# harukaki/brl

Measured on AMD Instinct MI355X. Metric: env-steps/sec at num_envs=8192, 32-step rollout, 1/2/4/8 MI355X, higher is better.
Workload: dtype u8

## Files before the change

brl_amd/csrc/brl_mlp_gemm_x3.hip:

```cpp
#include <hip/hip_runtime.h>
#include <stdint.h>

#include "abi_common.hpp"
#include "mlp_gemm_x3.hpp"
#include "mlp_linear_x3p.hpp"

static int64_t x3_tiles(int64_t m, int64_t n) { return ((m + 127) / 128) * ((n + 127) / 128); }

static int64_t x3_workspace_bytes(int64_t m, int64_t n, int64_t k) {
  const int sk = mgs::pick_splitk(m, n, k);
  if (sk == 1) return 0;
  const int64_t tiles = x3_tiles(m, n);
  return ((tiles * 4 + 255) / 256) * 256 + tiles * sk * (int64_t)mgs::SLAB_FLOATS * 4;
}

extern "C" int brl_mlp_gemm_x3_workspace(int64_t m, int64_t n, int64_t k, int64_t *bytes) {
  NEED(bytes && m > 0 && n > 0 && k > 0, "bytes / m / n / k");
  *bytes = x3_workspace_bytes(m, n, k);
  return BRL_OK;
}

extern "C" int brl_mlp_gemm_x3(int device, int layout, int epilogue, const float *a, int64_t lda, const float *b, int64_t ldb, float *c,
                               int64_t ldc, int64_t m, int64_t n, int64_t k, int act, const float *bias, const float *gate, int64_t ldg,
                               float *colsum, void *workspace, int64_t workspace_bytes, void *stream) {
  NEED(a && b && c && m > 0 && n > 0 && k > 0, "a / b / c / m / n / k");
  NEED(layout >= BRL_GEMM_NT && layout <= BRL_GEMM_TN, "layout (BRL_GEMM_NT / _NN / _TN)");
  NEED(m < (1 << 24) && n < (1 << 24) && k < (1 << 24), "m / n / k below 2^24");
  NEED(n % 4 == 0 && ldc % 4 == 0 && lda % 4 == 0 && ldb % 4 == 0 && ldc >= n, "n and the leading dimensions multiples of 4 (16-byte pieces)");
  const bool akc = layout != BRL_GEMM_TN, bkc = layout == BRL_GEMM_NT;
  NEED(k % 32 == 0, "k a multiple of 32 (whole 32-deep chunks; other k: brl_mlp_gemm)");
  NEED(akc ? lda >= k : lda >= ((m + 3) & ~(int64_t)3), "lda (where m is contiguous in a: at least m rounded up to 4 — whole 16-byte pieces are read)");
  NEED(bkc ? ldb >= k : ldb >= n, "ldb");
  NEED((akc ? m * lda : k * lda) < (1ll << 29) && (bkc ? n * ldb : k * ldb) < (1ll << 29), "operands below 2 GB");
  NEED(act == 0 || act == 1, "act (0 ReLU, 1 tanh)");
  NEED((epilogue == BRL_GEMM_EPI_NONE) || (epilogue == BRL_GEMM_EPI_BIAS_ACT && layout == BRL_GEMM_NT && bias) ||
           (epilogue == BRL_GEMM_EPI_GATE_COLSUM && layout == BRL_GEMM_NN && gate && ldg >= n && ldg % 4 == 0),
       "epilogue (NONE; BIAS_ACT with NT + bias; GATE_COLSUM with NN + gate)");
  NEED((((uintptr_t)a | (uintptr_t)b | (uintptr_t)c | (uintptr_t)bias | (uintptr_t)gate | (uintptr_t)colsum) & 15) == 0, "16-byte alignment");
  HIP_TRY(hipSetDevice(device));
  mgs::Args X{};
  mg::Args &G = X.g;
  G.A = a; G.lda = lda; G.B = b; G.ldb = ldb; G.C = c; G.ldc = ldc;
  G.M = (int)m; G.N = (int)n; G.K = (int)k; G.act = act;
  G.bias = bias; G.gate = gate; G.ldg = ldg; G.colsum = colsum;
  const int64_t tiles = x3_tiles(m, n);
  int sk = mgs::pick_splitk(m, n, k);
  const int64_t tick = ((tiles * 4 + 255) / 256) * 256;
  if (sk > 1 && (workspace == nullptr || workspace_bytes < tick + tiles * sk * (int64_t)mgs::SLAB_FLOATS * 4)) sk = 1;
  NEED(sk == 1 || (((uintptr_t)workspace) & 255) == 0, "workspace: 256-byte alignment");
  NEED(sk == 1 || tiles * sk * (int64_t)mgs::SLAB_FLOATS * 4 < (1ll << 31), "partial tiles below 2 GB");
  X.splitk = sk;
  X.tickets = (unsigned *)workspace;
  X.slabs = sk > 1 ? (float *)((char *)workspace + tick) : nullptr;
  const unsigned blocks = (unsigned)(tiles * sk);
  hipStream_t s = (hipStream_t)stream;
#define X3_LAUNCH(AK, BK_, E) hipLaunchKernelGGL((mgs::k_gemm_x3s<AK, BK_, E>), dim3(blocks), dim3(mgs::THREADS), 0, s, X)
  if (layout == BRL_GEMM_NT) {
    if (epilogue == BRL_GEMM_EPI_BIAS_ACT) X3_LAUNCH(true, true, mg::EPI_BIAS_ACT);
    else X3_LAUNCH(true, true, mg::EPI_NONE);
  } else if (layout == BRL_GEMM_NN) {
    if (epilogue == BRL_GEMM_EPI_GATE_COLSUM) X3_LAUNCH(true, false, mg::EPI_GATE_COLSUM);
    else X3_LAUNCH(true, false, mg::EPI_NONE);
  } else {
    X3_LAUNCH(false, false, mg::EPI_NONE);
  }
#undef X3_LAUNCH
  HIP_TRY(hipGetLastError());
  return BRL_OK;
}

extern "C" int brl_mlp_gemm_x3_group(int device, int layout, int count, const float *const *a, const int64_t *lda, const float *const *b,
                                     const int64_t *ldb, float *const *c, const int64_t *ldc, const int64_t *m, const int64_t *n,
                                     const int64_t *k, void *stream) {
  NEED(count >= 1 && count <= mgs::GROUP_MAX && a && lda && b && ldb && c && ldc && m && n && k, "count (1..8) / NULL array");
  NEED(layout >= BRL_GEMM_NT && layout <= BRL_GEMM_TN, "layout (BRL_GEMM_NT / _NN / _TN)");
  const bool akc = layout != BRL_GEMM_TN, bkc = layout == BRL_GEMM_NT;
  mgs::GroupArgs GA{};
  GA.n = count;
  for (int i = 0; i < count; i++) {
    NEED(a[i] && b[i] && c[i] && m[i] > 0 && n[i] > 0 && k[i] > 0, "a / b / c / m / n / k");
    NEED(m[i] < (1 << 24) && n[i] < (1 << 24) && k[i] < (1 << 24), "m / n / k below 2^24");
    NEED(n[i] % 4 == 0 && ldc[i] % 4 == 0 && lda[i] % 4 == 0 && ldb[i] % 4 == 0 && ldc[i] >= n[i], "n and the leading dimensions multiples of 4");
    NEED(k[i] % 32 == 0, "k a multiple of 32 (whole 32-deep chunks; other k: brl_mlp_gemm_group)");
    NEED(akc ? lda[i] >= k[i] : lda[i] >= ((m[i] + 3) & ~(int64_t)3), "lda (where m is contiguous in a: at least m rounded up to 4)");
    NEED(bkc ? ldb[i] >= k[i] : ldb[i] >= n[i], "ldb");
    NEED((akc ? m[i] * lda[i] : k[i] * lda[i]) < (1ll << 29) && (bkc ? n[i] * ldb[i] : k[i] * ldb[i]) < (1ll << 29), "operands below 2 GB");
    NEED((((uintptr_t)a[i] | (uintptr_t)b[i] | (uintptr_t)c[i]) & 15) == 0, "16-byte alignment");
    mgs::Args &X = GA.x[i];
    mg::Args &G = X.g;
    G.A = a[i]; G.lda = lda[i]; G.B = b[i]; G.ldb = ldb[i]; G.C = c[i]; G.ldc = ldc[i];
    G.M = (int)m[i]; G.N = (int)n[i]; G.K = (int)k[i];
    X.splitk = 1;
    GA.first[i + 1] = GA.first[i] + (int)x3_tiles(m[i], n[i]);
  }
  HIP_TRY(hipSetDevice(device));
  hipStream_t s = (hipStream_t)stream;
  const unsigned blocks = (unsigned)GA.first[count];
  if (layout == BRL_GEMM_NT) hipLaunchKernelGGL((mgs::k_gemm_x3s_group<true, true>), dim3(blocks), dim3(mgs::THREADS), 0, s, GA);
  else if (layout == BRL_GEMM_NN) hipLaunchKernelGGL((mgs::k_gemm_x3s_group<true, false>), dim3(blocks), dim3(mgs::THREADS), 0, s, GA);
  else hipLaunchKernelGGL((mgs::k_gemm_x3s_group<false, false>), dim3(blocks), dim3(mgs::THREADS), 0, s, GA);
  HIP_TRY(hipGetLastError());
  return BRL_OK;
}

extern "C" int brl_split_planes(int device, const float *x, int64_t n, uint16_t *planes, int64_t plane_stride, void *stream) {
  NEED(x && planes && n > 0 && n % 4 == 0 && plane_stride >= n && plane_stride % 4 == 0, "x / planes / n (a multiple of 4) / plane_stride");
  NEED((((uintptr_t)x) & 15) == 0 && (((uintptr_t)planes) & 7) == 0, "alignment (x 16 bytes, planes 8)");
  HIP_TRY(hipSetDevice(device));
  hipLaunchKernelGGL(lx3::k_split_planes, dim3((unsigned)((n / 4 + 255) / 256)), dim3(256), 0, (hipStream_t)stream, x, planes, plane_stride, n / 4);
  HIP_TRY(hipGetLastError());
  return BRL_OK;
}

extern "C" int brl_linear_x3p(int device, const uint16_t *x_planes, int npx, int64_t ldx, int64_t sx, const uint16_t *w_planes, int64_t ldw,
                              int64_t sw, const float *bias, int relu, float *y, int64_t ldy, uint16_t *y_planes, int64_t ldyp, int64_t syp,
                              int64_t m, int64_t n, int64_t k, void *stream) {
  NEED(x_planes && w_planes && bias && (y || y_planes) && m > 0 && n > 0 && k > 0, "x_planes / w_planes / bias / an output / m / n / k");
  NEED(npx == 1 || npx == 3, "npx (3 planes, or 1: x exact in bf16)");
  NEED(n % 128 == 0 && k % 32 == 0, "n a multiple of 128, k a multiple of 32");
  NEED(m < (1 << 24) && n < (1 << 24) && k < (1 << 24), "m / n / k below 2^24");
  NEED(ldx >= k && ldx % 8 == 0 && ldw >= k && ldw % 8 == 0, "ldx / ldw (at least k, multiples of 8: 16-byte pieces)");
  NEED(m * ldx < (1ll << 31) && n * ldw < (1ll << 31), "planes below 4 GB each");
  NEED(!y || (ldy >= n && ldy % 4 == 0), "ldy");
  NEED(!y_planes || (ldyp >= n && ldyp % 8 == 0 && syp % 8 == 0), "ldyp / syp (multiples of 8)");
  NEED(sx % 8 == 0 && sw % 8 == 0, "plane strides multiples of 8");
  NEED((((uintptr_t)x_planes | (uintptr_t)w_planes | (uintptr_t)bias | (uintptr_t)y | (uintptr_t)y_planes) & 15) == 0, "16-byte alignment");
  HIP_TRY(hipSetDevice(device));
  lx3::Args G{};
  G.x = x_planes; G.ldx = ldx; G.sx = sx; G.w = w_planes; G.ldw = ldw; G.sw = sw; G.bias = bias;
  G.y = y; G.ldy = ldy; G.yp = y_planes; G.ldyp = ldyp; G.syp = syp;
  G.M = (int)m; G.N = (int)n; G.K = (int)k; G.relu = relu ? 1 : 0;
  hipStream_t s = (hipStream_t)stream;
  const unsigned blocks = (unsigned)(((m + 127) / 128) * (n / 128));
  if (npx == 3) hipLaunchKernelGGL(lx3::k_linear_x3p<3>, dim3(blocks), dim3(lx3::THREADS), 0, s, G);
  else hipLaunchKernelGGL(lx3::k_linear_x3p<1>, dim3(blocks), dim3(lx3::THREADS), 0, s, G);
  HIP_TRY(hipGetLastError());
  return BRL_OK;
}
```

brl_amd/csrc/mlp_linear_x3p.hpp:

```cpp
#pragma once

#include "mlp_gemm.hpp"

namespace lx3 {

using mg::f32x4;
typedef __bf16 bf16x8 __attribute__((ext_vector_type(8)));
typedef float f32x16 __attribute__((ext_vector_type(16)));
typedef unsigned u32x4 __attribute__((ext_vector_type(4)));
typedef unsigned u32x2 __attribute__((ext_vector_type(2)));

constexpr int BK = 32, STAGES = 3, THREADS = 512;
constexpr int PLANE = 128 * 64;
constexpr int STAGE_BYTES = 6 * PLANE;
constexpr int LDS_BYTES = STAGES * STAGE_BYTES;
constexpr int C_ROW_BYTES = 128 * 2 + 16;
static_assert(3 * 128 * C_ROW_BYTES <= LDS_BYTES, "the output planes reuse the stages");

struct Args {
  const uint16_t *x;
  int64_t ldx, sx;
  const uint16_t *w;
  int64_t ldw, sw;
  const float *bias;
  float *y;
  int64_t ldy;
  uint16_t *yp;
  int64_t ldyp, syp;
  int M, N, K;
  int relu;
#ifdef LX3_TIMING
  unsigned long long *dbg;
#endif
};
#ifdef LX3_TIMING
#define LX3_STAMP(k) do { if (threadIdx.x == 0 && G.dbg) { G.dbg[(size_t)blockIdx.x * 4 + 2 * (k)] = __builtin_amdgcn_s_memtime(); \
                                                          G.dbg[(size_t)blockIdx.x * 4 + 2 * (k) + 1] = __builtin_amdgcn_s_memrealtime(); } } while (0)
#else
#define LX3_STAMP(k) do { } while (0)
#endif

template <bool V>
struct BoolTag { static constexpr bool value = V; };

#ifndef LX3_STORE
#define LX3_STORE 0
#endif
#ifndef LX3_EXP
#define LX3_EXP 0
#endif

__device__ __forceinline__ void glds16(const void *g, void *lds_wave_base) {
  __builtin_amdgcn_global_load_lds((const __attribute__((address_space(1))) void *)g, (__attribute__((address_space(3))) void *)lds_wave_base, 16,
                                   0, 0);
}

__device__ __forceinline__ void split3(const float x, unsigned &hi, unsigned &mid, unsigned &lo) {
  const unsigned u = __float_as_uint(x);
  const float r = x - __uint_as_float(u & 0xffff0000u);
  const unsigned ur = __float_as_uint(r);
  const float l = r - __uint_as_float(ur & 0xffff0000u);
  hi = u >> 16;
  mid = ur >> 16;
  lo = __float_as_uint(l) >> 16;
}

template <int NPX>
__global__ __launch_bounds__(THREADS) void k_linear_x3p(Args G) {
  static_assert(NPX == 1 || NPX == 3, "x: one plane (exact in bf16) or three");
  constexpr int NI = NPX + 3;
  constexpr int NP = NPX == 3 ? 6 : 3;
  constexpr int NMF = 4 * NP;
  constexpr int NFR = 2 * NPX + 3;
  __shared__ __attribute__((aligned(16))) unsigned char lds[LDS_BYTES];
  const int tid = (int)threadIdx.x, lane = tid & 63, w = __builtin_amdgcn_readfirstlane(tid >> 6);
  const int tiles_m = (G.M + 127) / 128, tiles_n = G.N / 128, nblk = (int)gridDim.x, bid = (int)blockIdx.x;
  const int L = (nblk % 8 == 0) ? (bid % 8) * (nblk / 8) + bid / 8 : bid;
  int tm, tn;
  if (tiles_m % 2 == 0 && tiles_n % 4 == 0) {
    const int blk = L >> 3, i = L & 7;
    tm = 2 * (blk / (tiles_n / 4)) + (i >> 2);
    tn = 4 * (blk % (tiles_n / 4)) + (i & 3);
  } else {
    tm = L / tiles_n;
    tn = L - tm * tiles_n;
  }
  const int m0 = tm * 128, n0 = tn * 128;
  const int nchunks = G.K / BK;

  uint32_t offx, offw;
  {
    const int row = 16 * w + (lane >> 2), pc = (lane & 3) ^ ((row >> 2) & 3);
    const int mr = (m0 + row < G.M) ? m0 + row : G.M - 1;
    offx = (uint32_t)(((int64_t)mr * G.ldx + 8 * pc) * 2);
    offw = (uint32_t)(((int64_t)(n0 + row) * G.ldw + 8 * pc) * 2);
  }
  int kc = 0;
  auto stage_one = [&](unsigned char *st, int j) __attribute__((always_inline)) {
    const bool isw = j >= NPX;
    const char *base = reinterpret_cast<const char *>(isw ? G.w + (int64_t)(j - NPX) * G.sw : G.x + (int64_t)j * G.sx);
    uint32_t o = (isw ? offw : offx) + (uint32_t)kc * (BK * 2);
    asm volatile("" : "+v"(o));
    glds16(base + o, st + j * PLANE + w * 1024);
  };

  const int wm = w >> 2, wn = w & 3, r32 = lane & 31, hh = lane >> 5;
  const int sw4 = (r32 >> 2) & 3;
  const int fa0 = (64 * wm + r32) * 64 + ((hh ^ sw4) << 4), fb0 = NPX * PLANE + (32 * wn + r32) * 64 + ((hh ^ sw4) << 4);
  auto read_frag = [&](const unsigned char *st, int s, int u) __attribute__((always_inline)) -> bf16x8 {
    const int off = (u < 2 * NPX) ? (u % NPX) * PLANE + (u / NPX) * 2048 + fa0 : (u - 2 * NPX) * PLANE + fb0;
    return __builtin_bit_cast(bf16x8, *reinterpret_cast<const u32x4 *>(st + (off ^ (s << 5))));
  };

  f32x16 acc[2][2];
#pragma unroll
  for (int b = 0; b < 2; b++)
#pragma unroll
    for (int c = 0; c < 2; c++)
#pragma unroll
      for (int e = 0; e < 16; e++) acc[b][c][e] = 0.0f;
  auto mf = [&](const bf16x8 (&f)[2][NFR], int t) __attribute__((always_inline)) {
    const int s = t / (2 * NP), u = t % (2 * NP), p = u >> 1, b = u & 1;
    int px, pw;
    if (NPX == 3) {
      px = (p == 0 || p == 3 || p == 5) ? 0 : (p == 2 || p == 4) ? 1 : 2;
      pw = (p == 1 || p == 4 || p == 5) ? 0 : (p == 2 || p == 3) ? 1 : 2;
    } else {
      px = 0;
      pw = 2 - p;
    }
    const int cls = (px == 0 && pw == 0) ? 0 : 1;
    if (!(LX3_EXP & 2)) acc[b][cls] = __builtin_amdgcn_mfma_f32_32x32x16_bf16(f[s][2 * NPX + pw], f[s][b * NPX + px], acc[b][cls], 0, 0, 0);
  };
  auto rorder = [&](int q, int &s, int &u) __attribute__((always_inline)) {
    s = q / NFR;
    const int i = q % NFR;
    if (NPX == 3) {
      constexpr int O[9] = {8, 0, 3, 6, 2, 5, 7, 1, 4};
      u = O[i];
    } else {
      constexpr int O[5] = {4, 0, 1, 3, 2};
      u = O[i];
    }
  };

  for (int c = 0; c < 2 && c < nchunks; c++) {
#pragma unroll
    for (int j = 0; j < NI; j++) stage_one(lds + c * STAGE_BYTES, j);
    kc++;
  }
  if (nchunks >= 2) {
    if (NI == 6) asm volatile("s_waitcnt vmcnt(6)" ::: "memory");
    else asm volatile("s_waitcnt vmcnt(4)" ::: "memory");
  } else {
    asm volatile("s_waitcnt vmcnt(0)" ::: "memory");
  }
  __builtin_amdgcn_s_barrier();
  asm volatile("" ::: "memory");
  if (nchunks >= 3) {
#pragma unroll
    for (int j = 0; j < NI; j++) stage_one(lds + 2 * STAGE_BYTES, j);
    kc++;
  }
  LX3_STAMP(0);
  bf16x8 f0[2][NFR], f1[2][NFR];
#pragma unroll
  for (int q = 0; q < 2 * NFR; q++) {
    int s, u;
    rorder(q, s, u);
    f0[s][u] = read_frag(lds, s, u);
  }

  auto phase = [&](auto full_tag, const bf16x8 (&fu)[2][NFR], bf16x8 (&fn)[2][NFR], int c, int stage) __attribute__((always_inline)) {
    constexpr bool FULL = decltype(full_tag)::value;
    const bool next = FULL || c + 1 < nchunks;
    const bool dma = (LX3_EXP & 1) ? false : (FULL || c + 3 < nchunks);
    unsigned char *st = lds + stage * STAGE_BYTES;
    const unsigned char *sn = lds + ((stage + 1 == STAGES) ? 0 : stage + 1) * STAGE_BYTES;
    __builtin_amdgcn_sched_barrier(0);
    mf(fu, 0);
    __builtin_amdgcn_sched_barrier(0);
    if (next) {
      if (FULL || c + 2 < nchunks) {
        if (NI == 6) asm volatile("s_waitcnt vmcnt(6) lgkmcnt(0)" ::: "memory");
        else asm volatile("s_waitcnt vmcnt(4) lgkmcnt(0)" ::: "memory");
      } else {
        asm volatile("s_waitcnt vmcnt(0) lgkmcnt(0)" ::: "memory");
      }
      if (!(LX3_EXP & 8)) __builtin_amdgcn_s_barrier();
      asm volatile("" ::: "memory");
    }
    __builtin_amdgcn_sched_barrier(0);
#pragma unroll
    for (int t = 1; t < NMF; t++) {
      mf(fu, t);
      __builtin_amdgcn_sched_barrier(0);
      if (t - 1 < NI && dma) stage_one(st, t - 1);
      if (t - 1 < 2 * NFR && next && !(LX3_EXP & 4)) {
        int s, u;
        rorder(t - 1, s, u);
        fn[s][u] = read_frag(sn, s, u);
      }
      __builtin_amdgcn_sched_barrier(0);
    }
    if (dma) kc++;
  };
  static_assert(2 * NFR <= NMF - 1, "a fragment read per gap");
  {
    using T = BoolTag<true>;
    using F = BoolTag<false>;
    const int nfull = nchunks - 3;
    int c = 0, stage = 0;
    auto nxt = [&]() { stage = (stage + 1 == STAGES) ? 0 : stage + 1; };
    for (; c + 1 < nfull; c += 2) {
      phase(T{}, f0, f1, c, stage); nxt();
      phase(T{}, f1, f0, c + 1, stage); nxt();
    }
    for (; c + 1 < nchunks; c += 2) {
      phase(F{}, f0, f1, c, stage); nxt();
      phase(F{}, f1, f0, c + 1, stage); nxt();
    }
    if (c < nchunks) phase(F{}, f0, f1, c, stage);
  }

  LX3_STAMP(1);
  __syncthreads();
  const float floor_v = G.relu ? 0.0f : -__builtin_inff();
#pragma unroll
  for (int b = 0; b < 2; b++) {
    const int row = 64 * wm + 32 * b + r32, em = m0 + row;
#pragma unroll
    for (int g = 0; g < 4; g++) {
      const int col = 32 * wn + 8 * g + 4 * hh;
      const f32x4 bias4 = *reinterpret_cast<const f32x4 *>(G.bias + n0 + col);
      f32x4 o;
#pragma unroll
      for (int e = 0; e < 4; e++) o[e] = fmaxf((acc[b][1][4 * g + e] + acc[b][0][4 * g + e]) + bias4[e], floor_v);
      if (G.y != nullptr && em < G.M) *reinterpret_cast<f32x4 *>(G.y + (int64_t)em * G.ldy + n0 + col) = o;
      if (G.yp != nullptr) {
        unsigned h[4], m[4], l[4];
#pragma unroll
        for (int e = 0; e < 4; e++) split3(o[e], h[e], m[e], l[e]);
        unsigned char *p = lds + row * C_ROW_BYTES + col * 2;
        *reinterpret_cast<u32x2 *>(p) = u32x2{h[0] | (h[1] << 16), h[2] | (h[3] << 16)};
        *reinterpret_cast<u32x2 *>(p + 128 * C_ROW_BYTES) = u32x2{m[0] | (m[1] << 16), m[2] | (m[3] << 16)};
        *reinterpret_cast<u32x2 *>(p + 2 * 128 * C_ROW_BYTES) = u32x2{l[0] | (l[1] << 16), l[2] | (l[3] << 16)};
      }
    }
  }
  if (G.yp != nullptr) {
    __syncthreads();
#pragma unroll
    for (int it = 0; it < (3 * 128 * 16) / THREADS; it++) {
      const int idx = it * THREADS + tid, pl = idx >> 11, row = (idx >> 4) & 127, ch = idx & 15;
      const u32x4 v = *reinterpret_cast<const u32x4 *>(lds + (pl * 128 + row) * C_ROW_BYTES + ch * 16);
      if (m0 + row < G.M) {
        u32x4 *dst = reinterpret_cast<u32x4 *>(G.yp + (int64_t)pl * G.syp + (int64_t)(m0 + row) * G.ldyp + n0 + ch * 8);
#if LX3_STORE == 1
        __builtin_nontemporal_store(v, dst);
#elif LX3_STORE == 2
        asm volatile("global_store_dwordx4 %0, %1, off sc0 sc1" ::"v"(dst), "v"(v) : "memory");
#else
        *dst = v;
#endif
      }
    }
  }
}

__global__ __launch_bounds__(256) void k_split_planes(const float *x, uint16_t *planes, int64_t stride, int64_t n4) {
  const int64_t idx = (int64_t)blockIdx.x * 256 + threadIdx.x;
  if (idx >= n4) return;
  const f32x4 v = reinterpret_cast<const f32x4 *>(x)[idx];
  unsigned h[4], m[4], l[4];
#pragma unroll
  for (int e = 0; e < 4; e++) split3(v[e], h[e], m[e], l[e]);
  uint16_t *p = planes + 4 * idx;
  *reinterpret_cast<u32x2 *>(p) = u32x2{h[0] | (h[1] << 16), h[2] | (h[3] << 16)};
  *reinterpret_cast<u32x2 *>(p + stride) = u32x2{m[0] | (m[1] << 16), m[2] | (m[3] << 16)};
  *reinterpret_cast<u32x2 *>(p + 2 * stride) = u32x2{l[0] | (l[1] << 16), l[2] | (l[3] << 16)};
}

}
```

Baseline: 10.73 billion.

## Make linear_x3p kernel persistent and prefetch next tile during epilogue

The grid for the x3p linear kernel is capped at the compute-unit count (overridable by env var), and each block loops over several output tiles. The first two k-chunks of the next tile are requested before the current tile's epilogue, so loads overlap with bias/activation, plane splitting and stores. When a next tile follows, the output planes are staged one plane at a time through the freed stage. This adds waitcnt bookkeeping for pending stores, extra barriers, and uses fewer concurrent blocks per CU, which can reduce latency hiding.

```diff
diff --git a/brl_amd/csrc/brl_mlp_gemm_x3.hip b/brl_amd/csrc/brl_mlp_gemm_x3.hip
--- a/brl_amd/csrc/brl_mlp_gemm_x3.hip
+++ b/brl_amd/csrc/brl_mlp_gemm_x3.hip
@@ -1,5 +1,8 @@
 #include <hip/hip_runtime.h>
 #include <stdint.h>
+#include <stdlib.h>
+
+#include <atomic>
 
 #include "abi_common.hpp"
 #include "mlp_gemm_x3.hpp"
@@ -112,6 +115,16 @@
   return BRL_OK;
 }
 
+static hipError_t lx3_compute_units(int device, int *cus) {
+  static std::atomic<int> cached[64];
+  const bool slot = device >= 0 && device < 64;
+  *cus = slot ? cached[device].load(std::memory_order_relaxed) : 0;
+  if (*cus > 0) return hipSuccess;
+  const hipError_t err = hipDeviceGetAttribute(cus, hipDeviceAttributeMultiprocessorCount, device);
+  if (err == hipSuccess && slot) cached[device].store(*cus, std::memory_order_relaxed);
+  return err;
+}
+
 extern "C" int brl_linear_x3p(int device, const uint16_t *x_planes, int npx, int64_t ldx, int64_t sx, const uint16_t *w_planes, int64_t ldw,
                               int64_t sw, const float *bias, int relu, float *y, int64_t ldy, uint16_t *y_planes, int64_t ldyp, int64_t syp,
                               int64_t m, int64_t n, int64_t k, void *stream) {
@@ -131,7 +144,16 @@
   G.y = y; G.ldy = ldy; G.yp = y_planes; G.ldyp = ldyp; G.syp = syp;
   G.M = (int)m; G.N = (int)n; G.K = (int)k; G.relu = relu ? 1 : 0;
   hipStream_t s = (hipStream_t)stream;
-  const unsigned blocks = (unsigned)(((m + 127) / 128) * (n / 128));
+  const int64_t tiles = ((m + 127) / 128) * (n / 128);
+  const char *e = getenv("BRL_LX3_GRID");
+  const int64_t forced = e ? atoll(e) : 0;
+  int64_t cap = forced;
+  if (forced <= 0) {
+    int cus = 0;
+    HIP_TRY(lx3_compute_units(device, &cus));
+    cap = cus > 0 ? cus : tiles;
+  }
+  const unsigned blocks = (unsigned)(tiles < cap ? tiles : cap);
   if (npx == 3) hipLaunchKernelGGL(lx3::k_linear_x3p<3>, dim3(blocks), dim3(lx3::THREADS), 0, s, G);
   else hipLaunchKernelGGL(lx3::k_linear_x3p<1>, dim3(blocks), dim3(lx3::THREADS), 0, s, G);
   HIP_TRY(hipGetLastError());
diff --git a/brl_amd/csrc/mlp_linear_x3p.hpp b/brl_amd/csrc/mlp_linear_x3p.hpp
--- a/brl_amd/csrc/mlp_linear_x3p.hpp
+++ b/brl_amd/csrc/mlp_linear_x3p.hpp
@@ -15,7 +15,7 @@
 constexpr int STAGE_BYTES = 6 * PLANE;
 constexpr int LDS_BYTES = STAGES * STAGE_BYTES;
 constexpr int C_ROW_BYTES = 128 * 2 + 16;
-static_assert(3 * 128 * C_ROW_BYTES <= LDS_BYTES, "the output planes reuse the stages");
+static_assert(3 * 128 * C_ROW_BYTES <= LDS_BYTES && 128 * C_ROW_BYTES <= STAGE_BYTES, "the output planes reuse the stages: all three, or one plane in one stage");
 
 struct Args {
   const uint16_t *x;
@@ -34,14 +34,16 @@
 #endif
 };
 #ifdef LX3_TIMING
-#define LX3_STAMP(k) do { if (threadIdx.x == 0 && G.dbg) { G.dbg[(size_t)blockIdx.x * 4 + 2 * (k)] = __builtin_amdgcn_s_memtime(); \
-                                                          G.dbg[(size_t)blockIdx.x * 4 + 2 * (k) + 1] = __builtin_amdgcn_s_memrealtime(); } } while (0)
+#define LX3_STAMP(k) do { if (threadIdx.x == 0 && G.dbg) { G.dbg[(size_t)blockIdx.x * 8 + 2 * (k)] = __builtin_amdgcn_s_memtime(); \
+                                                          G.dbg[(size_t)blockIdx.x * 8 + 2 * (k) + 1] = __builtin_amdgcn_s_memrealtime(); } } while (0)
 #else
 #define LX3_STAMP(k) do { } while (0)
 #endif
 
 template <bool V>
 struct BoolTag { static constexpr bool value = V; };
+template <int V>
+struct IntTag { static constexpr int value = V; };
 
 #ifndef LX3_STORE
 #define LX3_STORE 0
@@ -53,6 +55,21 @@
 __device__ __forceinline__ void glds16(const void *g, void *lds_wave_base) {
   __builtin_amdgcn_global_load_lds((const __attribute__((address_space(1))) void *)g, (__attribute__((address_space(3))) void *)lds_wave_base, 16,
                                    0, 0);
+}
+
+__device__ __forceinline__ void wait_vm(int n) {
+#define LX3_WAIT(N) case N: asm volatile("s_waitcnt vmcnt(" #N ") lgkmcnt(0)" ::: "memory"); break;
+  switch (n) {
+    LX3_WAIT(4) LX3_WAIT(6) LX3_WAIT(8) LX3_WAIT(12) LX3_WAIT(14) LX3_WAIT(16) LX3_WAIT(18) LX3_WAIT(20) LX3_WAIT(24) LX3_WAIT(26)
+    default: asm volatile("s_waitcnt vmcnt(0) lgkmcnt(0)" ::: "memory"); break;
+  }
+#undef LX3_WAIT
+}
+
+__device__ __forceinline__ void lds_barrier() {
+  asm volatile("s_waitcnt lgkmcnt(0)" ::: "memory");
+  __builtin_amdgcn_s_barrier();
+  asm volatile("" ::: "memory");
 }
 
 __device__ __forceinline__ void split3(const float x, unsigned &hi, unsigned &mid, unsigned &lo) {
@@ -74,28 +91,34 @@
   constexpr int NFR = 2 * NPX + 3;
   __shared__ __attribute__((aligned(16))) unsigned char lds[LDS_BYTES];
   const int tid = (int)threadIdx.x, lane = tid & 63, w = __builtin_amdgcn_readfirstlane(tid >> 6);
-  const int tiles_m = (G.M + 127) / 128, tiles_n = G.N / 128, nblk = (int)gridDim.x, bid = (int)blockIdx.x;
-  const int L = (nblk % 8 == 0) ? (bid % 8) * (nblk / 8) + bid / 8 : bid;
-  int tm, tn;
-  if (tiles_m % 2 == 0 && tiles_n % 4 == 0) {
-    const int blk = L >> 3, i = L & 7;
-    tm = 2 * (blk / (tiles_n / 4)) + (i >> 2);
-    tn = 4 * (blk % (tiles_n / 4)) + (i & 3);
-  } else {
-    tm = L / tiles_n;
-    tn = L - tm * tiles_n;
-  }
-  const int m0 = tm * 128, n0 = tn * 128;
+  const int tiles_m = (G.M + 127) / 128, tiles_n = G.N / 128, ntiles = tiles_m * tiles_n, nblk = (int)gridDim.x;
+  int t = (int)blockIdx.x;
+  if (t >= ntiles) return;
   const int nchunks = G.K / BK;
-
-  uint32_t offx, offw;
-  {
+  auto place = [&](int tt, int &m0_, int &n0_) __attribute__((always_inline)) {
+    const int L = (ntiles % 8 == 0) ? (tt % 8) * (ntiles / 8) + tt / 8 : tt;
+    int tm, tn;
+    if (tiles_m % 2 == 0 && tiles_n % 4 == 0) {
+      const int blk = L >> 3, i = L & 7;
+      tm = 2 * (blk / (tiles_n / 4)) + (i >> 2);
+      tn = 4 * (blk % (tiles_n / 4)) + (i & 3);
+    } else {
+      tm = L / tiles_n;
+      tn = L - tm * tiles_n;
+    }
+    m0_ = tm * 128;
+    n0_ = tn * 128;
+  };
+
+  uint32_t offx = 0, offw = 0;
+  int kc = 0;
+  auto aim = [&](int m0_, int n0_) __attribute__((always_inline)) {
     const int row = 16 * w + (lane >> 2), pc = (lane & 3) ^ ((row >> 2) & 3);
-    const int mr = (m0 + row < G.M) ? m0 + row : G.M - 1;
+    const int mr = (m0_ + row < G.M) ? m0_ + row : G.M - 1;
     offx = (uint32_t)(((int64_t)mr * G.ldx + 8 * pc) * 2);
-    offw = (uint32_t)(((int64_t)(n0 + row) * G.ldw + 8 * pc) * 2);
-  }
-  int kc = 0;
+    offw = (uint32_t)(((int64_t)(n0_ + row) * G.ldw + 8 * pc) * 2);
+    kc = 0;
+  };
   auto stage_one = [&](unsigned char *st, int j) __attribute__((always_inline)) {
     const bool isw = j >= NPX;
     const char *base = reinterpret_cast<const char *>(isw ? G.w + (int64_t)(j - NPX) * G.sw : G.x + (int64_t)j * G.sx);
@@ -103,6 +126,14 @@
     asm volatile("" : "+v"(o));
     glds16(base + o, st + j * PLANE + w * 1024);
   };
+  auto request_two = [&](int s0) __attribute__((always_inline)) {
+    for (int c = 0; c < 2 && c < nchunks; c++) {
+      const int si = (s0 + c >= STAGES) ? s0 + c - STAGES : s0 + c;
+#pragma unroll
+      for (int j = 0; j < NI; j++) stage_one(lds + si * STAGE_BYTES, j);
+      kc++;
+    }
+  };
 
   const int wm = w >> 2, wn = w & 3, r32 = lane & 31, hh = lane >> 5;
   const int sw4 = (r32 >> 2) & 3;
@@ -113,14 +144,8 @@
   };
 
   f32x16 acc[2][2];
-#pragma unroll
-  for (int b = 0; b < 2; b++)
-#pragma unroll
-    for (int c = 0; c < 2; c++)
-#pragma unroll
-      for (int e = 0; e < 16; e++) acc[b][c][e] = 0.0f;
-  auto mf = [&](const bf16x8 (&f)[2][NFR], int t) __attribute__((always_inline)) {
-    const int s = t / (2 * NP), u = t % (2 * NP), p = u >> 1, b = u & 1;
+  auto mf = [&](const bf16x8 (&f)[2][NFR], int t_) __attribute__((always_inline)) {
+    const int s = t_ / (2 * NP), u = t_ % (2 * NP), p = u >> 1, b = u & 1;
     int px, pw;
     if (NPX == 3) {
       px = (p == 0 || p == 3 || p == 5) ? 0 : (p == 2 || p == 4) ? 1 : 2;
@@ -144,35 +169,18 @@
     }
   };
 
-  for (int c = 0; c < 2 && c < nchunks; c++) {
-#pragma unroll
-    for (int j = 0; j < NI; j++) stage_one(lds + c * STAGE_BYTES, j);
-    kc++;
-  }
-  if (nchunks >= 2) {
-    if (NI == 6) asm volatile("s_waitcnt vmcnt(6)" ::: "memory");
-    else asm volatile("s_waitcnt vmcnt(4)" ::: "memory");
-  } else {
-    asm volatile("s_waitcnt vmcnt(0)" ::: "memory");
-  }
-  __builtin_amdgcn_s_barrier();
-  asm volatile("" ::: "memory");
-  if (nchunks >= 3) {
-#pragma unroll
-    for (int j = 0; j < NI; j++) stage_one(lds + 2 * STAGE_BYTES, j);
-    kc++;
-  }
-  LX3_STAMP(0);
+  int m0, n0;
+  place(t, m0, n0);
+  aim(m0, n0);
+  request_two(0);
+  int base = 0;
+  int pend = 0;
+  bool follows = false;
+  (void)follows;
   bf16x8 f0[2][NFR], f1[2][NFR];
-#pragma unroll
-  for (int q = 0; q < 2 * NFR; q++) {
-    int s, u;
-    rorder(q, s, u);
-    f0[s][u] = read_frag(lds, s, u);
-  }
-
-  auto phase = [&](auto full_tag, const bf16x8 (&fu)[2][NFR], bf16x8 (&fn)[2][NFR], int c, int stage) __attribute__((always_inline)) {
-    constexpr bool FULL = decltype(full_tag)::value;
+
+  auto phase = [&](auto full_tag, auto first_tag, const bf16x8 (&fu)[2][NFR], bf16x8 (&fn)[2][NFR], int c, int stage) __attribute__((always_inline)) {
+    constexpr bool FULL = decltype(full_tag)::value, FIRST = decltype(first_tag)::value;
     const bool next = FULL || c + 1 < nchunks;
     const bool dma = (LX3_EXP & 1) ? false : (FULL || c + 3 < nchunks);
     unsigned char *st = lds + stage * STAGE_BYTES;
@@ -180,8 +188,11 @@
     __builtin_amdgcn_sched_barrier(0);
     mf(fu, 0);
     __builtin_amdgcn_sched_barrier(0);
+    if (FIRST && follows) LX3_STAMP(3);
     if (next) {
-      if (FULL || c + 2 < nchunks) {
+      if (FIRST) {
+        wait_vm(((c + 2 < nchunks) ? NI : 0) + pend);
+      } else if (FULL || c + 2 < nchunks) {
         if (NI == 6) asm volatile("s_waitcnt vmcnt(6) lgkmcnt(0)" ::: "memory");
         else asm volatile("s_waitcnt vmcnt(4) lgkmcnt(0)" ::: "memory");
       } else {
@@ -192,13 +203,13 @@
     }
     __builtin_amdgcn_sched_barrier(0);
 #pragma unroll
-    for (int t = 1; t < NMF; t++) {
-      mf(fu, t);
+    for (int t_ = 1; t_ < NMF; t_++) {
+      mf(fu, t_);
       __builtin_amdgcn_sched_barrier(0);
-      if (t - 1 < NI && dma) stage_one(st, t - 1);
-      if (t - 1 < 2 * NFR && next && !(LX3_EXP & 4)) {
+      if (t_ - 1 < NI && dma) stage_one(st, t_ - 1);
+      if (t_ - 1 < 2 * NFR && next && !(LX3_EXP & 4)) {
         int s, u;
-        rorder(t - 1, s, u);
+        rorder(t_ - 1, s, u);
         fn[s][u] = read_frag(sn, s, u);
       }
       __builtin_amdgcn_sched_barrier(0);
@@ -206,65 +217,135 @@
     if (dma) kc++;
   };
   static_assert(2 * NFR <= NMF - 1, "a fragment read per gap");
-  {
-    using T = BoolTag<true>;
-    using F = BoolTag<false>;
-    const int nfull = nchunks - 3;
-    int c = 0, stage = 0;
-    auto nxt = [&]() { stage = (stage + 1 == STAGES) ? 0 : stage + 1; };
-    for (; c + 1 < nfull; c += 2) {
-      phase(T{}, f0, f1, c, stage); nxt();
-      phase(T{}, f1, f0, c + 1, stage); nxt();
-    }
-    for (; c + 1 < nchunks; c += 2) {
-      phase(F{}, f0, f1, c, stage); nxt();
-      phase(F{}, f1, f0, c + 1, stage); nxt();
-    }
-    if (c < nchunks) phase(F{}, f0, f1, c, stage);
-  }
-
-  LX3_STAMP(1);
-  __syncthreads();
-  const float floor_v = G.relu ? 0.0f : -__builtin_inff();
-#pragma unroll
-  for (int b = 0; b < 2; b++) {
-    const int row = 64 * wm + 32 * b + r32, em = m0 + row;
-#pragma unroll
-    for (int g = 0; g < 4; g++) {
-      const int col = 32 * wn + 8 * g + 4 * hh;
-      const f32x4 bias4 = *reinterpret_cast<const f32x4 *>(G.bias + n0 + col);
-      f32x4 o;
-#pragma unroll
-      for (int e = 0; e < 4; e++) o[e] = fmaxf((acc[b][1][4 * g + e] + acc[b][0][4 * g + e]) + bias4[e], floor_v);
-      if (G.y != nullptr && em < G.M) *reinterpret_cast<f32x4 *>(G.y + (int64_t)em * G.ldy + n0 + col) = o;
-      if (G.yp != nullptr) {
+
+  auto store_planes = [&](auto per_tag, unsigned char *buf, const u32x2 (&pk)[3][2][4], int er32, int ehh, int etid) __attribute__((always_inline)) {
+    constexpr int PER = decltype(per_tag)::value;
+#pragma unroll
+    for (int p0 = 0; p0 < 3; p0 += PER) {
+      if (p0 > 0) lds_barrier();
+#pragma unroll
+      for (int q = 0; q < PER; q++)
+#pragma unroll
+        for (int b = 0; b < 2; b++)
+#pragma unroll
+          for (int g = 0; g < 4; g++)
+            *reinterpret_cast<u32x2 *>(buf + (q * 128 + 64 * wm + 32 * b + er32) * C_ROW_BYTES + (32 * wn + 8 * g + 4 * ehh) * 2) = pk[p0 + q][b][g];
+      lds_barrier();
+#pragma unroll
+      for (int it = 0; it < (PER * 128 * 16) / THREADS; it++) {
+        const int idx = it * THREADS + etid, q = idx >> 11, row = (idx >> 4) & 127, ch = idx & 15;
+        const u32x4 v = *reinterpret_cast<const u32x4 *>(buf + (q * 128 + row) * C_ROW_BYTES + ch * 16);
+        if (m0 + row < G.M) {
+          u32x4 *dst = reinterpret_cast<u32x4 *>(G.yp + (int64_t)(p0 + q) * G.syp + (int64_t)(m0 + row) * G.ldyp + n0 + ch * 8);
+#if LX3_STORE == 1
+          __builtin_nontemporal_store(v, dst);
+#elif LX3_STORE == 2
+          asm volatile("global_store_dwordx4 %0, %1, off sc0 sc1" ::"v"(dst), "v"(v) : "memory");
+#else
+          *dst = v;
+#endif
+        }
+      }
+    }
+  };
+
+  for (;;) {
+#pragma unroll
+    for (int b = 0; b < 2; b++)
+#pragma unroll
+      for (int c = 0; c < 2; c++)
+#pragma unroll
+        for (int e = 0; e < 16; e++) acc[b][c][e] = 0.0f;
+
+    wait_vm(((nchunks >= 2) ? NI : 0) + pend);
+    __builtin_amdgcn_s_barrier();
+    asm volatile("" ::: "memory");
+    if (nchunks >= 3) {
+      const int s2 = (base + 2 >= STAGES) ? base + 2 - STAGES : base + 2;
+#pragma unroll
+      for (int j = 0; j < NI; j++) stage_one(lds + s2 * STAGE_BYTES, j);
+      kc++;
+    }
+    LX3_STAMP(0);
+#pragma unroll
+    for (int q = 0; q < 2 * NFR; q++) {
+      int s, u;
+      rorder(q, s, u);
+      f0[s][u] = read_frag(lds + base * STAGE_BYTES, s, u);
+    }
+
+    {
+      using T = BoolTag<true>;
+      using F = BoolTag<false>;
+      const int nfull = nchunks - 3;
+      int c = 1, stage = base;
+      auto nxt = [&]() { stage = (stage + 1 == STAGES) ? 0 : stage + 1; };
+      phase(F{}, T{}, f0, f1, 0, stage); nxt();
+      for (; c + 1 < nfull; c += 2) {
+        phase(T{}, F{}, f1, f0, c, stage); nxt();
+        phase(T{}, F{}, f0, f1, c + 1, stage); nxt();
+      }
+      for (; c + 1 < nchunks; c += 2) {
+        phase(F{}, F{}, f1, f0, c, stage); nxt();
+        phase(F{}, F{}, f0, f1, c + 1, stage); nxt();
+      }
+      if (c < nchunks) phase(F{}, F{}, f1, f0, c, stage);
+    }
+    LX3_STAMP(1);
+
+    const bool more = t + nblk < ntiles;
+    const int sl = (base + nchunks - 1) % STAGES;
+    int le = lane;
+    asm volatile("" : "+v"(le));
+    const int er32 = le & 31, ehh = le >> 5, etid = 64 * w + le;
+    float bias_w[32];
+    {
+      const __attribute__((address_space(4))) float *bp = (const __attribute__((address_space(4))) float *)(G.bias + n0 + 32 * wn);
+#pragma unroll
+      for (int i = 0; i < 32; i++) bias_w[i] = bp[i];
+    }
+    int m1 = 0, n1 = 0;
+    if (more) {
+      t += nblk;
+      place(t, m1, n1);
+      aim(m1, n1);
+      request_two(sl + 1 == STAGES ? 0 : sl + 1);
+    }
+    asm volatile("" ::: "memory");
+    __builtin_amdgcn_sched_barrier(0);
+
+    if (G.yp != nullptr) lds_barrier();
+    const float floor_v = G.relu ? 0.0f : -__builtin_inff();
+    u32x2 pk[3][2][4];
+#pragma unroll
+    for (int b = 0; b < 2; b++) {
+      const int em = m0 + 64 * wm + 32 * b + er32;
+#pragma unroll
+      for (int g = 0; g < 4; g++) {
+        const int col = 32 * wn + 8 * g + 4 * ehh;
+        f32x4 o;
+#pragma unroll
+        for (int e = 0; e < 4; e++) o[e] = fmaxf((acc[b][1][4 * g + e] + acc[b][0][4 * g + e]) + (ehh ? bias_w[8 * g + 4 + e] : bias_w[8 * g + e]), floor_v);
+        if (G.y != nullptr && em < G.M) *reinterpret_cast<f32x4 *>(G.y + (int64_t)em * G.ldy + n0 + col) = o;
         unsigned h[4], m[4], l[4];
 #pragma unroll
         for (int e = 0; e < 4; e++) split3(o[e], h[e], m[e], l[e]);
-        unsigned char *p = lds + row * C_ROW_BYTES + col * 2;
-        *reinterpret_cast<u32x2 *>(p) = u32x2{h[0] | (h[1] << 16), h[2] | (h[3] << 16)};
-        *reinterpret_cast<u32x2 *>(p + 128 * C_ROW_BYTES) = u32x2{m[0] | (m[1] << 16), m[2] | (m[3] << 16)};
-        *reinterpret_cast<u32x2 *>(p + 2 * 128 * C_ROW_BYTES) = u32x2{l[0] | (l[1] << 16), l[2] | (l[3] << 16)};
-      }
-    }
-  }
-  if (G.yp != nullptr) {
-    __syncthreads();
-#pragma unroll
-    for (int it = 0; it < (3 * 128 * 16) / THREADS; it++) {
-      const int idx = it * THREADS + tid, pl = idx >> 11, row = (idx >> 4) & 127, ch = idx & 15;
-      const u32x4 v = *reinterpret_cast<const u32x4 *>(lds + (pl * 128 + row) * C_ROW_BYTES + ch * 16);
-      if (m0 + row < G.M) {
-        u32x4 *dst = reinterpret_cast<u32x4 *>(G.yp + (int64_t)pl * G.syp + (int64_t)(m0 + row) * G.ldyp + n0 + ch * 8);
-#if LX3_STORE == 1
-        __builtin_nontemporal_store(v, dst);
-#elif LX3_STORE == 2
-        asm volatile("global_store_dwordx4 %0, %1, off sc0 sc1" ::"v"(dst), "v"(v) : "memory");
-#else
-        *dst = v;
-#endif
-      }
-    }
+        pk[0][b][g] = u32x2{h[0] | (h[1] << 16), h[2] | (h[3] << 16)};
+        pk[1][b][g] = u32x2{m[0] | (m[1] << 16), m[2] | (m[3] << 16)};
+        pk[2][b][g] = u32x2{l[0] | (l[1] << 16), l[2] | (l[3] << 16)};
+      }
+    }
+    if (G.yp != nullptr) {
+      if (more) store_planes(IntTag<1>{}, lds + sl * STAGE_BYTES, pk, er32, ehh, etid);
+      else store_planes(IntTag<3>{}, lds, pk, er32, ehh, etid);
+    }
+    if (!more) break;
+    LX3_STAMP(2);
+    pend = (m0 + 128 <= G.M) ? (G.y != nullptr ? 8 : 0) + (G.yp != nullptr ? 12 : 0) : 0;
+    m0 = m1;
+    n0 = n1;
+    base = (sl + 1 == STAGES) ? 0 : sl + 1;
+    follows = true;
   }
 }
 
```

New measurement: 10.71 billion. No clear change (-0.2%).
